# askerlee/segtran

Measured on AMD Instinct MI355X. Metric: train-step images/sec (cfg2, re-associated op order), higher is better.
Workload: dtype f32; 1 GPU; REFUGE fundus 2D, segtran eff-b4, translayers 3, layercompress 1,1,2,2, 512x512, bs 6/GPU; global_batch=6, per_gpu_batch=6, parallelism=dp1, step=fwd+BCE/Dice+bwd+allreduce+clip+BertAdam, op_order=re-associated, ranks=1

## Files before the change

include/segx.h:

```cpp
#ifndef SEGX_H
#define SEGX_H
#include <stdint.h>
#ifdef __cplusplus
extern "C" {
#endif

int segx_version(void);
int segx_last_error(char* buf, int buflen);

enum { SEGX_EPI_NONE = 0, SEGX_EPI_GELU = 1 ,
       SEGX_EPI_SWISH = 2  };
enum { SEGX_BIAS_NONE = 0, SEGX_BIAS_N = 1 , SEGX_BIAS_M = 2  };
enum { SEGX_ENGINE_F32 = 0, SEGX_ENGINE_BF16X6 = 1 };
enum { SEGX_ENGINE_SEL_DEFAULT = 0, SEGX_ENGINE_SEL_F32 = 1, SEGX_ENGINE_SEL_BF16X6 = 2 };
enum { SEGX_TILE_AUTO = 0, SEGX_TILE_128x128 = 1, SEGX_TILE_64x64 = 2, SEGX_TILE_128x32 = 3, SEGX_TILE_32x128 = 4, SEGX_TILE_64x128 = 5,
       SEGX_TILE_256x128 = 6, SEGX_TILE_WS128x128 = 7, SEGX_TILE_WS128x256 = 8, SEGX_TILE_WS64x256 = 9,
       SEGX_TILE_WS96x256 = 10, SEGX_TILE_WS256x96 = 11,
       SEGX_TILE_SKINNY_NT = 12   };
typedef struct {
    int32_t M, N, K, nb0, nb1;
    int64_t a_b0, a_b1, a_m, a_k;
    int64_t b_b0, b_b1, b_n, b_k;
    int64_t c_b0, c_b1, c_m;
    float alpha;
    int32_t epilogue, bias_mode;
    int64_t bias_b1;
    const float* bias;
    float* aux;
    float* gmax;
    float dropout_p;
    uint64_t seed, offset;
    int32_t splitk;
    float* workspace;
    int32_t tile;
    int64_t bias_b0;
    int32_t batch_reduce;
    int32_t engine;
    const void* b_planes;
    int64_t bp_b0, bp_b1;
    const float* resid;
} segx_gemm_desc;
int segx_gemm_f32(const float* A, const float* B, float* C, const segx_gemm_desc* d, void* stream);
int segx_gemm_plan(const float* A, const float* B, const segx_gemm_desc* d, int* tile, int* splitk);
int segx_gemm_plan_model(const float* A, const float* B, const segx_gemm_desc* d, int* tile, int* splitk);
int segx_gemm_route(const float* A, const float* B, const segx_gemm_desc* d, int32_t* out);
int64_t segx_x6_presplit_elems(int rows, int K, int nb0, int nb1);
int segx_x6_presplit(const float* W, int rows, int K, int64_t s_row, int64_t s_k, int nb0, int nb1, int64_t s_b0, int64_t s_b1, void* planes, void* stream);


int segx_softmax_fwd(const float* S, float* P, float* Pdrop, int64_t rows, int L, float clip, const float* gmax,
                     float p, uint64_t seed, uint64_t offset, void* stream);
// ... 229 lines not shown
```

segtran_amd/csrc/common.h:

```cpp
#pragma once
#include <hip/hip_runtime.h>
#include <stdint.h>
#include <stdio.h>
#include <stdarg.h>
#include <string.h>
#include <math.h>
#include <atomic>
#include "../../include/segx.h"

typedef float f32x16 __attribute__((ext_vector_type(16)));
typedef float f32x4 __attribute__((ext_vector_type(4)));

namespace segx {

inline char* err_buf() { static thread_local char buf[512] = {0}; return buf; }
inline int fail(int code, const char* fmt, ...) {
    va_list ap; va_start(ap, fmt); vsnprintf(err_buf(), 512, fmt, ap); va_end(ap); return code;
}
inline int check_launch(const char* what) {
    hipError_t e = hipGetLastError();
    if (e != hipSuccess) return fail((int)e, "%s: %s", what, hipGetErrorString(e));
    return 0;
}
#ifndef SEGX_MIN_WAVES_PER_SIMD
// ... 175 lines not shown
    s = odd2 ? v[0] : v[2]; r = SEGX_QUAD_XOR(s, 2); v[0] = odd2 ? r : v[0]; v[2] = odd2 ? v[2] : r;
    s = odd2 ? v[1] : v[3]; r = SEGX_QUAD_XOR(s, 2); v[1] = odd2 ? r : v[1]; v[3] = odd2 ? v[3] : r;
}
__device__ __forceinline__ float dropout_scale(uint64_t seed, uint64_t offset, uint64_t idx, float p, float inv_keep) {
    const u32x4 r = philox4(seed, (offset + idx) >> 2);
    const unsigned sel = (unsigned)((offset + idx) & 3);
    const unsigned u = sel == 0 ? r.x : sel == 1 ? r.y : sel == 2 ? r.z : r.w;
    return keep_of(u, p, inv_keep);
}

__device__ __forceinline__ float swish_fwd(float x) { return x * (1.0f / (1.0f + __expf(-x))); }
__device__ __forceinline__ float gelu_erf(float x) { return 0.5f * x * (1.0f + erff(x * 0.70710678118654752440f)); }
__device__ __forceinline__ float gelu_erf_grad(float x) {
    const float cdf = 0.5f * (1.0f + erff(x * 0.70710678118654752440f));
    const float pdf = 0.39894228040143267794f * __expf(-0.5f * x * x);
    return cdf + x * pdf;
}

#define SEGX_KNOB_TABLE(X)                                                                                                                                        \
    X(1, interp_variant, 0, 0, 2)                                                                  \
    X(2, conv_small_policy, 0, 0, 1)                          \
    X(3, bn_path, 0, 0, 2)                            \
    X(4, engine, SEGX_ENGINE_F32, SEGX_ENGINE_F32, SEGX_ENGINE_BF16X6)                                                                   \
    X(6, x6_variant, 0, 0, 7)                                      \
    X(7, conv_x6_wgrad_all, 0, 0, 2)                  \
    X(8, dw_strip_outputs, 8192, 256, 2147483647)                                                         \
    X(9, ws_grid, 256, 8, 4096)                                                                         \
    X(12, team_spin, (int)TEAM_SPIN_LIMIT, 32, 1 << 24)                                                     \
    X(13, team_drop, 0, 0, 4096)                      \
    X(14, pool_slab, 0, 0, 2)                         \
    X(15, pool_dslide, 1, 0, 1)                       \
    X(16, conv_halo, 1, 0, 1)                         \
    X(17, conv_halo_min_tiles, 256, 1, 1 << 24)         \
    X(18, skinny_nt, 1, 0, 1)                         \
    X(19, tile_walk, 1, 0, 1)                         \
    X(20, x6_terms, 6, 3, 6)
struct Knobs {
#define SEGX_KNOB_FIELD(id, field, def, lo, hi) std::atomic<int> field{def};
    SEGX_KNOB_TABLE(SEGX_KNOB_FIELD)
#undef SEGX_KNOB_FIELD
    std::atomic<int> x6_launches{0};
    std::atomic<int> x3_launches{0};
};
inline Knobs& knobs() { static Knobs k; return k; }
inline int kget(const std::atomic<int>& a) { return a.load(std::memory_order_relaxed); }

inline const uint64_t*& rng_base() { static const uint64_t* p = nullptr; return p; }

inline int ceil_div(int64_t a, int64_t b) { return (int)((a + b - 1) / b); }
__device__ __forceinline__ unsigned xcd_block(unsigned b, unsigned n) {
    const unsigned q = n >> 3, r = n & 7, xcd = b & 7, idx = b >> 3;
    return (xcd < r ? xcd * (q + 1) : r * (q + 1) + (xcd - r) * q) + idx;
}
__host__ __device__ inline int64_t i64min(int64_t a, int64_t b) { return a < b ? a : b; }
__host__ __device__ inline int64_t i64max(int64_t a, int64_t b) { return a > b ? a : b; }

struct FastDiv { unsigned d, magic; };
__host__ __device__ inline FastDiv make_fastdiv(int d) { FastDiv f; f.d = (unsigned)d; f.magic = d <= 1 ? 0u : (unsigned)(((1ull << 32) + d - 1) / d); return f; }
__device__ __forceinline__ int fdiv(int n, const FastDiv& f) {
    if (f.d <= 1) return n;
    const unsigned q = __umulhi((unsigned)n, f.magic);
    return (int)(q - (q * f.d > (unsigned)n ? 1u : 0u));
}


}
```

segtran_amd/csrc/gemm.hip:

```cpp
#include "gemm_x6ws.h"
#include "gemm_skinny.h"
#include "gemm_tuned.h"

namespace segx {

template <class Cfg, bool AKC, bool BKC, bool VEC, int EPI>
__global__ __launch_bounds__(256, 2) void gemm_f32_kernel(GemmArgs g) {
    __shared__ __attribute__((aligned(16))) TileLdsT<Cfg> lds;
    const TileCoord t = tile_coord<Cfg>(g);
    const DenseLoader<AKC, VEC, Cfg::BM> la{g.A + t.z0 * g.a_b0 + t.z1 * g.a_b1, g.a_m, g.a_k, t.m0, g.M};
    const DenseLoader<BKC, VEC, Cfg::BN> lb{g.B + t.z0 * g.b_b0 + t.z1 * g.b_b1, g.b_n, g.b_k, t.n0, g.N};
    f32x16 acc[Cfg::MI][Cfg::NJ];
    gemm_mainloop<Cfg>(acc, la, lb, t.kbeg, t.kend, lds);
    gemm_epilogue<EPI, Cfg>(acc, g, t);
}

template <class Cfg, bool AKC, bool BKC, int EPI, int WPE, int VAR = 0, int TERMS = 6>
__global__ __launch_bounds__(256) SEGX_MIN_WAVES_PER_SIMD(WPE) void gemm_x6_kernel(GemmArgs g) {
    __shared__ __attribute__((aligned(16))) unsigned char lds[X6Lds<Cfg, TERMS>::BYTES];
    const TileCoord t = tile_coord<Cfg>(g);
    const DenseLoader6<AKC, Cfg::BM> la{g.A + t.z0 * g.a_b0 + t.z1 * g.a_b1, g.a_m, g.a_k, t.m0, g.M};
    const DenseLoader6<BKC, Cfg::BN> lb{g.B + t.z0 * g.b_b0 + t.z1 * g.b_b1, g.b_n, g.b_k, t.n0, g.N};
    f32x16 acc[Cfg::MI][Cfg::NJ];
    gemm_mainloop_x6<Cfg, DenseLoader6<AKC, Cfg::BM>, DenseLoader6<BKC, Cfg::BN>, VAR, TERMS>(acc, la, lb, t.kbeg, t.kend, lds);
    gemm_epilogue<EPI, Cfg>(acc, g, t);
}

template <class Cfg, bool AKC, bool BKC, int EPI, int WPE, int TERMS = 6>
__global__ __launch_bounds__(256) SEGX_MIN_WAVES_PER_SIMD(WPE) void gemm_x6_lean_kernel(GemmArgs g) {
    __shared__ __attribute__((aligned(16))) unsigned char lds[X6Lds<Cfg, TERMS>::BYTES];
    const TileCoord t = tile_coord<Cfg>(g);
    WsDense6<AKC, Cfg::BM> la; WsDense6<BKC, Cfg::BN> lb;
    la.begin(g.A + t.z0 * g.a_b0 + t.z1 * g.a_b1, g.a_m, g.a_k, t.m0, g.M, threadIdx.x);
    lb.begin(g.B + t.z0 * g.b_b0 + t.z1 * g.b_b1, g.b_n, g.b_k, t.n0, g.N, threadIdx.x);
// ... 87 lines not shown
        double t;
        const int sk = price(TileInfo{w6.id, w6.bm, w6.bn, w6.wg_per_cu, w6.ktile_us * fws, w6.fixed_us}, M, N, K, nbatch, may_split, splitk_fixed, kget(knobs().ws_grid), &t);
        if (t < best_t * 0.97) { best_t = t; *tile = w6.id; *splitk = sk; }
    }
}
static bool gemm_lean_ok(const segx_gemm_desc* d) {
    const bool akc = (d->a_k == 1), bkc = (d->b_k == 1);
    const int64_t a_span = akc ? (int64_t)d->M * d->a_m : (int64_t)d->K * d->a_k, b_span = bkc ? (int64_t)d->N * d->b_n : (int64_t)d->K * d->b_k;
    return d->K % BKT == 0 && a_span < (1LL << 29) && b_span < (1LL << 29);
}
static bool gemm_ws_ok(const segx_gemm_desc* d) { return !d->resid && gemm_lean_ok(d); }
static void plan(int M, int N, int K, int nbatch, bool vec, bool may_split, int splitk_fixed, int* tile, int* splitk, bool skinny_ok = true) {
    const TileInfo* cand[3]; int nc = 0;
    if (!vec) cand[nc++] = &kTiles[0];
    else if (skinny_ok && N <= 48 && M > N) cand[nc++] = &tile_info(SEGX_TILE_128x32);
    else if (skinny_ok && M <= 48) cand[nc++] = &tile_info(SEGX_TILE_32x128);
    else { cand[nc++] = &kTiles[0]; cand[nc++] = &kTiles[1]; cand[nc++] = &kTiles[2]; }
    double best_t = -1.0;
    for (int i = 0; i < nc; ++i) {
        double t;
        const int sk = price(*cand[i], M, N, K, nbatch, may_split, splitk_fixed, 0, &t);
        if (best_t < 0.0 || t < best_t * 0.97) { best_t = t; *tile = cand[i]->id; *splitk = sk; }
    }
}
static bool gemm_vec_ok(const float* A, const float* B, const segx_gemm_desc* d) {
    const bool akc = (d->a_k == 1), bkc = (d->b_k == 1);
    const bool vecA = aligned16(A) && (d->a_b0 % 4 == 0) && (d->a_b1 % 4 == 0) && ((akc ? d->a_m : d->a_k) % 4 == 0) &&
                      ((akc ? d->K : d->M) % 4 == 0);
    const bool vecB = aligned16(B) && (d->b_b0 % 4 == 0) && (d->b_b1 % 4 == 0) && ((bkc ? d->b_n : d->b_k) % 4 == 0) &&
                      ((bkc ? d->K : d->N) % 4 == 0);
    return vecA && vecB;
}
static int skinny_nt_splitk(const float* A, const float* B, const segx_gemm_desc* d) {
    if (!kget(knobs().skinny_nt) || !d->batch_reduce || d->epilogue != SEGX_EPI_NONE || d->gmax || d->resid || d->a_k != 1 || d->b_k != 1) return 0;
    if (!gemm_vec_ok(A, B, d)) return 0;
    const int nbatch = d->nb0 * d->nb1;
    const int sk = (int)i64max(1, (int64_t)kget(knobs().ws_grid) * skinny_nt_wgs_per_cu(d->M, d->N) / nbatch);
    if (!skinny_nt_shape_ok(d->M, d->N, d->K, nbatch, sk * nbatch)) return 0;
    if ((int64_t)d->M * d->a_m >= (1LL << 31) || (int64_t)d->N * d->b_n >= (1LL << 31)) return 0;
    return sk;
}

static int gemm_plan_impl(const float* A, const float* B, const segx_gemm_desc* d, int* tile, int* splitk, bool use_table) {
    SEGX_REQUIRE(A && B && d && tile && splitk && d->M > 0 && d->N > 0 && d->K > 0 && d->nb0 > 0 && d->nb1 > 0, "segx_gemm_plan: bad args");
    const bool plain = d->epilogue == SEGX_EPI_NONE, swish = d->epilogue == SEGX_EPI_SWISH;
    int t = SEGX_TILE_128x128, sk = 1;
    const bool vec = gemm_vec_ok(A, B, d);
    if (const int ssk = skinny_nt_splitk(A, B, d)) { *tile = SEGX_TILE_SKINNY_NT; *splitk = ssk; return 0; }
    if (use_table && plain && !d->gmax && x6_eligible(call_engine(d), d->M, d->N, vec)) {
        const int nbt = d->nb0 * d->nb1; const bool akc_ = d->a_k == 1, bkc_ = d->b_k == 1;
        for (const TunedGemm& e : kTunedGemm)
            if (e.M == d->M && e.N == d->N && e.K == d->K && e.nb == nbt && (e.akc != 0) == akc_ && (e.bkc != 0) == bkc_) {
                if (e.tile >= SEGX_TILE_256x128 && !gemm_ws_ok(d)) break;
                *tile = e.tile; *splitk = e.splitk;
                return 0;
            }
    }
    if (x6_eligible(call_engine(d), d->M, d->N, vec) && (plain || d->a_k == 1))
        plan6(d->M, d->N, d->K, d->nb0 * d->nb1, !plain && !swish, plain && !d->gmax, 0, gemm_ws_ok(d) && !swish, (d->a_k != 1) + (d->b_k != 1), &t, &sk);
    else plan(d->M, d->N, d->K, d->nb0 * d->nb1, vec && (plain || swish), plain && !d->gmax, 0, &t, &sk, !swish);
    *tile = t; *splitk = sk;
    return 0;
}

enum GemmFamily {
    GEMM_F32,
    GEMM_X6,
    GEMM_X6_LEAN,
    GEMM_WS,
    GEMM_WS_PRE,
    GEMM_SKINNY
};
struct GemmRoute {
    int family;
    int tile;
    bool akc, bkc;
    bool vec;
    int epi;
    int sched;
    int splitk;
    int ws_grid;
    bool walk;
    int terms;
};
static bool ws_tile_id(int tile) { return tile >= SEGX_TILE_256x128 && tile <= SEGX_TILE_WS256x96; }
static bool x3_built(const GemmRoute& r) {
    if (r.sched != 0) return false;
    const bool plain = r.epi == SEGX_EPI_NONE, conv = r.akc && !r.bkc;
    switch (r.family) {
        case GEMM_WS: return plain && r.akc && (r.tile != SEGX_TILE_WS64x256 || !r.bkc);
        case GEMM_X6: return conv && r.epi != SEGX_EPI_GELU;
        case GEMM_X6_LEAN:
            if (!plain) return r.akc;
            return conv || (r.bkc && (r.tile != SEGX_TILE_64x128 || !r.akc));
        default: return false;
    }
}

static int gemm_route(const float* A, const float* B, const segx_gemm_desc* d, GemmRoute* out) {
    GemmRoute r;
    r.akc = d->a_k == 1; r.bkc = d->b_k == 1; r.vec = gemm_vec_ok(A, B, d);
    r.epi = d->epilogue; r.sched = 0; r.splitk = d->splitk > 1 ? d->splitk : 1;
    r.ws_grid = kget(knobs().ws_grid); r.walk = kget(knobs().tile_walk) != 0; r.terms = 0;
    const int want_terms = kget(knobs().x6_terms);
    const int nbatch = d->nb0 * d->nb1;
    const bool gelu = d->epilogue == SEGX_EPI_GELU, swish = d->epilogue == SEGX_EPI_SWISH, ws_forced = ws_tile_id(d->tile);
    const int engine = call_engine(d);
    SEGX_REQUIRE(!ws_forced || engine == SEGX_ENGINE_BF16X6, "segx_gemm_f32: tile %d exists on the bf16x6 engine only", d->tile);
    int tile = d->tile;
    if (tile == SEGX_TILE_SKINNY_NT) {
        const int ssk = skinny_nt_splitk(A, B, d);
        if (ssk > 0 && r.splitk <= ssk) { r.family = GEMM_SKINNY; r.tile = tile; *out = r; return 0; }
        tile = SEGX_TILE_AUTO;
    }
    const bool ws_ok = gemm_ws_ok(d);
    const bool x6 = x6_eligible(engine, d->M, d->N, r.vec) && (!gelu || r.akc) &&
                    (tile == SEGX_TILE_AUTO || tile == SEGX_TILE_128x128 || tile == SEGX_TILE_64x128 || tile == SEGX_TILE_64x64 || ws_forced);
    if (tile == SEGX_TILE_AUTO) {
        int sk_unused = 1;
        if (x6) plan6(d->M, d->N, d->K, nbatch, gelu, false, r.splitk, ws_ok && !swish, (!r.akc) + (!r.bkc), &tile, &sk_unused);
        else plan(d->M, d->N, d->K, nbatch, r.vec && !gelu, false, r.splitk, &tile, &sk_unused, !swish);
    }
    if (swish && tile != SEGX_TILE_64x128 && tile != SEGX_TILE_64x64) tile = SEGX_TILE_128x128;
    if (ws_forced && !ws_ok) tile = SEGX_TILE_128x128;
    if ((tile == SEGX_TILE_WS96x256 && (!r.akc || gelu)) || (tile == SEGX_TILE_WS256x96 && (!r.bkc || gelu))) tile = SEGX_TILE_128x128;
    if (gelu && (tile == SEGX_TILE_WS128x256 || tile == SEGX_TILE_WS64x256)) tile = SEGX_TILE_128x128;
    const bool ws = x6 && ws_ok && ws_tile_id(tile);
    if (!r.vec || (gelu && !ws) || (ws_forced && !x6)) tile = SEGX_TILE_128x128;
    r.tile = tile;
    if (!x6) {
        SEGX_REQUIRE(!gelu || r.akc, "segx_gemm_f32: the GELU epilogue is built for a k-contiguous A operand (nn.Linear, attention fusion)");
        r.family = GEMM_F32;
    } else if (ws) {
        const int v = kget(knobs().x6_variant);
        r.sched = v == 1 ? 1 : 0;
#ifdef SEGX_BENCH
        if (v >= 2 && v <= 5 && !gelu && r.akc && r.bkc) r.sched = v;
#endif
        const bool pre = d->b_planes && !gelu && (tile == SEGX_TILE_256x128 || tile == SEGX_TILE_WS128x256);
        r.family = pre ? GEMM_WS_PRE : GEMM_WS;
        if (pre) r.sched = 0;
    } else {
        const int v = kget(knobs().x6_variant);
        if (v > 0 && !gelu && r.akc && r.bkc && tile == SEGX_TILE_128x128) {
            r.family = GEMM_X6; r.sched = v;
// ... 151 lines not shown
        case GEMM_WS: return ws_kernel(r);
        case GEMM_WS_PRE: return r.tile == SEGX_TILE_256x128 ? ws_pre_tile<Cfg256x128>(r) : ws_pre_tile<Cfg128x256>(r);
        default: return f32_kernel(r);
    }
}
static void set_tiles(GemmArgs& g, const GemmLaunch& k, const GemmRoute& r) {
    g.tiles_m = ceil_div(g.M, k.bm); g.tiles_n = ceil_div(g.N, k.bn); g.mfast = r.walk ? tile_walk(g.M, g.N, g.K, g.tiles_m) : 0;
}
static int persistent_grid(const GemmArgs& g, const GemmRoute& r, int* grid) {
    const int64_t items = (int64_t)g.tiles_m * g.tiles_n * g.nbatch * g.splitk;
    SEGX_REQUIRE(items < 2147483647LL - 512, "segx_gemm_f32: too many tiles");
    *grid = (int)i64min(r.ws_grid, (items + 7) / 8 * 8);
    return 0;
}
static void slab_reduce(const segx_gemm_desc* d, float* C, const float* bias, int nslabs, bool skinny, hipStream_t stream) {
    const int64_t total = (int64_t)d->M * d->N;
    const float* ws = static_cast<const float*>(d->workspace);
    if (total * 16 <= 512 * 1024 && nslabs >= 16)
        hipLaunchKernelGGL((slab_sum_parts_kernel<16>), dim3((unsigned)((total + 15) / 16)), dim3(256), 0, stream, ws, C, bias, d->M, d->N, nslabs, total, d->c_m, d->alpha, d->bias_mode);
    else if (skinny || (total * 4 <= 1024 * 1024 && nslabs >= 4))
        hipLaunchKernelGGL((slab_sum_parts_kernel<4>), dim3((unsigned)((total + 63) / 64)), dim3(256), 0, stream, ws, C, bias, d->M, d->N, nslabs, total, d->c_m, d->alpha, d->bias_mode);
    else
        SEGX_SPLITK_REDUCE((unsigned)i64min(2048, (total + 255) / 256), stream, ws, C, bias, d->M, d->N, 1, nslabs, total, (int64_t)0, (int64_t)0, d->c_m, d->alpha,
                           d->bias_mode, (int64_t)0, (int64_t)0, total, (const float*)nullptr);
}
}

extern "C" int segx_gemm_plan(const float* A, const float* B, const segx_gemm_desc* d, int* tile, int* splitk) { return segx::gemm_plan_impl(A, B, d, tile, splitk, true); }
extern "C" int segx_gemm_plan_model(const float* A, const float* B, const segx_gemm_desc* d, int* tile, int* splitk) { return segx::gemm_plan_impl(A, B, d, tile, splitk, false); }

extern "C" int segx_gemm_route(const float* A, const float* B, const segx_gemm_desc* d, int32_t* out) {
    using namespace segx;
    SEGX_REQUIRE(A && B && d && out && d->M > 0 && d->N > 0 && d->K > 0 && d->nb0 > 0 && d->nb1 > 0, "segx_gemm_route: bad args");
    SEGX_REQUIRE(d->tile >= SEGX_TILE_AUTO && d->tile <= SEGX_TILE_SKINNY_NT && d->engine >= SEGX_ENGINE_SEL_DEFAULT && d->engine <= SEGX_ENGINE_SEL_BF16X6,
                 "segx_gemm_route: bad tile %d or engine selector %d", d->tile, d->engine);
    GemmRoute r;
    const int rc = gemm_route(A, B, d, &r);
    if (rc) return rc;
    out[0] = r.family; out[1] = r.tile; out[2] = r.terms; out[3] = r.splitk;
    return 0;
}

extern "C" int segx_gemm_f32(const float* A, const float* B, float* C, const segx_gemm_desc* d, void* stream_) {
    using namespace segx;
    hipStream_t stream = (hipStream_t)stream_;
    SEGX_REQUIRE(A && B && C && d, "segx_gemm_f32: null pointer");
    SEGX_REQUIRE(d->M > 0 && d->N > 0 && d->K > 0 && d->nb0 > 0 && d->nb1 > 0, "segx_gemm_f32: bad sizes M=%d N=%d K=%d nb=%dx%d",
                 d->M, d->N, d->K, d->nb0, d->nb1);
    SEGX_REQUIRE(d->a_m == 1 || d->a_k == 1, "segx_gemm_f32: A needs a unit stride (a_m=%lld a_k=%lld)", (long long)d->a_m, (long long)d->a_k);
    SEGX_REQUIRE(d->b_n == 1 || d->b_k == 1, "segx_gemm_f32: B needs a unit stride (b_n=%lld b_k=%lld)", (long long)d->b_n, (long long)d->b_k);
    SEGX_REQUIRE(d->epilogue == SEGX_EPI_NONE || d->epilogue == SEGX_EPI_GELU || d->epilogue == SEGX_EPI_SWISH, "segx_gemm_f32: bad epilogue %d", d->epilogue);
    SEGX_REQUIRE(d->epilogue != SEGX_EPI_SWISH || (d->a_k == 1 && d->b_n == 1 && d->b_k != 1 && !d->resid && !d->gmax && d->dropout_p == 0.f),
                 "segx_gemm_f32: the swish epilogue is built for a pointwise convolution's forward (A k-contiguous, B row-contiguous; no resid, gmax or dropout)");
    SEGX_REQUIRE(d->epilogue != SEGX_EPI_GELU || d->aux, "segx_gemm_f32: GELU epilogue needs aux");
    SEGX_REQUIRE(d->bias_mode == SEGX_BIAS_NONE || d->bias, "segx_gemm_f32: bias_mode set but bias null");
    SEGX_REQUIRE(d->dropout_p >= 0.f && d->dropout_p < 1.f, "segx_gemm_f32: dropout_p out of range");
    const int splitk = d->splitk > 1 ? d->splitk : 1;
    SEGX_REQUIRE(splitk == 1 || (d->workspace && d->epilogue == SEGX_EPI_NONE && !d->gmax), "segx_gemm_f32: split-K needs workspace and a plain epilogue");
    const bool breduce = d->batch_reduce != 0;
    SEGX_REQUIRE(!breduce || (d->workspace && d->epilogue == SEGX_EPI_NONE && !d->gmax), "segx_gemm_f32: batch_reduce needs workspace and a plain epilogue");
    SEGX_REQUIRE(!d->resid || (d->epilogue == SEGX_EPI_NONE && !breduce && !d->gmax), "segx_gemm_f32: resid needs a plain epilogue (no GELU, no batch_reduce, no gmax)");
    SEGX_REQUIRE(d->tile >= SEGX_TILE_AUTO && d->tile <= SEGX_TILE_SKINNY_NT, "segx_gemm_f32: bad tile %d", d->tile);
    SEGX_REQUIRE(d->engine >= SEGX_ENGINE_SEL_DEFAULT && d->engine <= SEGX_ENGINE_SEL_BF16X6, "segx_gemm_f32: bad engine selector %d", d->engine);
    GemmRoute r;
    int rc = gemm_route(A, B, d, &r);
    if (rc) return rc;

    const int nbatch = d->nb0 * d->nb1;
    const float* bias = d->bias_mode ? d->bias : nullptr;
    if (r.family == GEMM_SKINNY) {
        const int nslabs = splitk * nbatch;
        rc = launch_skinny_nt(A, B, static_cast<float*>(d->workspace), d->M, d->N, d->K, d->nb0, d->nb1, d->a_b0, d->a_b1, d->a_m, d->b_b0, d->b_b1, d->b_n, nslabs, stream);
        if (rc) return rc;
        slab_reduce(d, C, bias, nslabs, true, stream);
        return check_launch("segx_gemm_f32/skinny_nt_reduce");
    }
    GemmArgs g;
    g.A = A; g.B = B; g.C = C; g.bias = bias; g.aux = d->epilogue == SEGX_EPI_GELU ? d->aux : nullptr;
    g.gmax = d->gmax;
    g.M = d->M; g.N = d->N; g.K = d->K; g.nb1 = d->nb1; g.nbatch = nbatch;
    g.a_b0 = d->a_b0; g.a_b1 = d->a_b1; g.a_m = d->a_m; g.a_k = d->a_k;
    g.b_b0 = d->b_b0; g.b_b1 = d->b_b1; g.b_n = d->b_n; g.b_k = d->b_k;
    g.c_b0 = d->c_b0; g.c_b1 = d->c_b1; g.c_m = d->c_m; g.bias_b1 = d->bias_b1; g.bias_b0 = d->bias_b0;
    g.alpha = d->alpha; g.epilogue = d->epilogue; g.bias_mode = d->bias_mode;
    g.vecA = r.vec; g.vecB = r.vec;
    g.dropout_p = d->dropout_p; g.seed = d->seed; g.offset = d->offset; g.rbase = rng_base();
    g.splitk = splitk;
    g.k_chunk = splitk == 1 ? d->K : ceil_div(ceil_div(d->K, splitk), BKT) * BKT;
    g.c_split = (int64_t)nbatch * d->M * d->N;
    g.slab = breduce ? 1 : 0;
    g.Bp = nullptr; g.bp_plane = g.bp_b0 = g.bp_b1 = 0;
    if (r.family == GEMM_WS_PRE) { g.Bp = static_cast<const unsigned short*>(d->b_planes); g.bp_plane = (int64_t)d->N * d->K; g.bp_b0 = d->bp_b0; g.bp_b1 = d->bp_b1; }
    g.resid = d->resid;
    if (splitk > 1 || breduce) g.C = d->workspace;

    if (r.family != GEMM_F32) knobs().x6_launches.fetch_add(1, std::memory_order_relaxed);
    if (r.terms == 3) knobs().x3_launches.fetch_add(1, std::memory_order_relaxed);
    const GemmLaunch k = route_kernel(r);
    set_tiles(g, k, r);
    if (r.family == GEMM_WS || r.family == GEMM_WS_PRE) {
        int grid;
        rc = persistent_grid(g, r, &grid);
        if (rc) return rc;
        hipLaunchKernelGGL(k.fn, dim3(grid), dim3(512), 0, stream, g);
    } else
        hipLaunchKernelGGL(k.fn, dim3(g.tiles_m * g.tiles_n, nbatch, splitk), dim3(256), 0, stream, g);
    rc = check_launch("segx_gemm_f32");
    if (rc) return rc;
    if (breduce) {
// ... 30 lines not shown
```

segtran_amd/segx.py:

```python
import contextlib
import ctypes
import enum
import os
import torch

_HERE = os.path.dirname(os.path.abspath(__file__))
LIB_PATH = os.path.join(_HERE, 'lib', 'libsegx.so')

c_f = ctypes.c_float
c_i = ctypes.c_int32
c_l = ctypes.c_int64
c_u = ctypes.c_uint64
c_p = ctypes.c_void_p


class GemmDesc(ctypes.Structure):
    _fields_ = [('M', c_i), ('N', c_i), ('K', c_i), ('nb0', c_i), ('nb1', c_i),
                ('a_b0', c_l), ('a_b1', c_l), ('a_m', c_l), ('a_k', c_l),
                ('b_b0', c_l), ('b_b1', c_l), ('b_n', c_l), ('b_k', c_l),
                ('c_b0', c_l), ('c_b1', c_l), ('c_m', c_l),
                ('alpha', c_f), ('epilogue', c_i), ('bias_mode', c_i), ('bias_b1', c_l),
                ('bias', c_p), ('aux', c_p), ('gmax', c_p),
                ('dropout_p', c_f), ('seed', c_u), ('offset', c_u),
                ('splitk', c_i), ('workspace', c_p), ('tile', c_i), ('bias_b0', c_l), ('batch_reduce', c_i), ('engine', c_i),
                ('b_planes', c_p), ('bp_b0', c_l), ('bp_b1', c_l), ('resid', c_p)]


EPI_NONE, EPI_GELU, EPI_SWISH = 0, 1, 2
(TILE_AUTO, TILE_128x128, TILE_64x64, TILE_128x32, TILE_32x128, TILE_64x128, TILE_256x128, TILE_WS128x128, TILE_WS128x256, TILE_WS64x256,
 TILE_WS96x256, TILE_WS256x96, TILE_SKINNY_NT) = range(13)
BIAS_NONE, BIAS_N, BIAS_M = 0, 1, 2


class Knob(enum.IntEnum):
    INTERP_VARIANT = 1
    CONV_SMALL_POLICY = 2
    BN_PATH = 3
    ENGINE = 4
    X6_LAUNCHES = 5
    X6_VARIANT = 6
    CONV_X6_WGRAD_ALL = 7
    DW_STRIP_OUTPUTS = 8
    WS_GRID = 9
    TEAM_SPIN = 12
    TEAM_DROP = 13
    POOL_SLAB = 14
    POOL_DSLIDE = 15
    CONV_HALO = 16
    CONV_HALO_MIN_TILES = 17
    SKINNY_NT = 18
    TILE_WALK = 19


Knob.X6_TERMS = 20


def knob_id(name):
    v = getattr(Knob, name.upper(), None)
    if not isinstance(v, int) or name.upper().startswith('_'):
        raise KeyError(name)
    return v


# ... 105 lines not shown
        d = GemmDesc()
        d.resid = _ptr(resid)
        d.M, d.N, d.K, d.nb0, d.nb1 = M, N, K, nb[0], nb[1]
        d.a_b0, d.a_b1, d.a_m, d.a_k = a_strides
        d.b_b0, d.b_b1, d.b_n, d.b_k = b_strides
        d.c_b0, d.c_b1, d.c_m = c_strides
        d.alpha, d.epilogue, d.bias_mode, d.bias_b1, d.bias_b0 = alpha, epilogue, bias_mode, bias_b1, bias_b0
        d.bias, d.aux, d.gmax = _ptr(bias), _ptr(aux), _ptr(gmax)
        d.dropout_p, d.seed, d.offset = dropout_p, seed, offset
        if b_planes is not None:
            self._chk_t(b_planes[0])
            d.b_planes, d.bp_b0, d.bp_b1 = _ptr(b_planes[0]), b_planes[1], b_planes[2]
        d.engine = 0 if engine is None else 1 + self.ENGINES[engine]
        d.batch_reduce = 1 if batch_reduce else 0
        if splitk == 0:
            t, sk = c_i(0), c_i(0)
            self.check(self.c.segx_gemm_plan(_ptr(A), _ptr(B), ctypes.byref(d), ctypes.byref(t), ctypes.byref(sk)), 'segx_gemm_plan')
            tile, splitk = t.value, sk.value
            workspace = torch.empty(splitk * nb[0] * nb[1] * M * N, dtype=torch.float32, device=C.device) if (splitk > 1 or batch_reduce) else None
        d.splitk, d.workspace = splitk, _ptr(workspace)
        d.tile = self.force_tile if self.force_tile is not None else tile
        if self.gemm_prof is not None and C.is_cuda:
            e0, e1 = torch.cuda.Event(enable_timing=True), torch.cuda.Event(enable_timing=True)
            self.x6_launches()
            e0.record()
            rc = self.c.segx_gemm_f32(_ptr(A), _ptr(B), _ptr(C), ctypes.byref(d), self.stream(C))
            e1.record()
            self.gemm_prof.append((e0, e1, 2.0 * M * N * K * nb[0] * nb[1], (M, N, K, nb[0] * nb[1], a_strides[3] == 1, b_strides[3] == 1, splitk, d.tile),
                                   self.x6_launches() > 0))
        else:
            rc = self.c.segx_gemm_f32(_ptr(A), _ptr(B), _ptr(C), ctypes.byref(d), self.stream(C))
        self.check(rc, 'segx_gemm_f32')

    ROUTE_FAMILIES = ('f32', 'x6', 'x6_lean', 'ws', 'ws_pre', 'skinny')

    def gemm_route(self, A, B, M, N, K, a_strides, b_strides, nb=(1, 1), epilogue=EPI_NONE, splitk=1, tile=TILE_AUTO, engine=None):
        self._chk_t(A, B)
        d = GemmDesc()
        d.M, d.N, d.K, d.nb0, d.nb1 = M, N, K, nb[0], nb[1]
        d.a_b0, d.a_b1, d.a_m, d.a_k = a_strides
        d.b_b0, d.b_b1, d.b_n, d.b_k = b_strides
        d.epilogue, d.splitk, d.tile = epilogue, splitk, tile
        d.engine = 0 if engine is None else 1 + self.ENGINES[engine]
        out = (c_i * 4)()
        self.check(self.c.segx_gemm_route(_ptr(A), _ptr(B), ctypes.byref(d), out), 'segx_gemm_route')
        return self.ROUTE_FAMILIES[out[0]], out[1], out[2], out[3]

    def x6_presplit(self, W, rows, K, s_row, s_k, nb=(1, 1), s_b=(0, 0)):
        e0, e1 = (nb[0] if s_b[0] else 1), (nb[1] if s_b[1] else 1)
        planes = torch.empty(self.c.segx_x6_presplit_elems(rows, K, e0, e1), dtype=torch.int16, device=W.device)
        self._chk_t(W)
        self.check(self.c.segx_x6_presplit(_ptr(W), rows, K, s_row, s_k, e0, e1, s_b[0], s_b[1], _ptr(planes), self.stream(W)), 'segx_x6_presplit')
        per = 3 * rows * K
        return planes, (e1 * per if s_b[0] else 0), (per if s_b[1] else 0)

    def _call(self, name, ref, *args):
        conv = []
        dev = None
        hip = not self.emulated
        for a in args:
            if isinstance(a, torch.Tensor):
                if hip and not a.is_cuda:
                    raise RuntimeError('libsegx (HIP) called with a CPU tensor')
                if dev is None:
                    dev = a.device
                elif a.device != dev:
                    raise AssertionError('tensors on different devices')
# ... 494 lines not shown
```

Before: 94.68 images/s.

## Add streaming GEMM kernel for small-M/small-K shapes with N-contiguous B

Adds a streaming GEMM path for shapes with a small M or K and a long N dimension. The whole A operand stays resident in LDS while waves stream 32-column strips of B through a register prefetch ring and issue fp32 MFMA. The planner selects it automatically when the shape is eligible, enabled by a new bit in the skinny_nt knob (default now 7). The goal is to avoid the padding and low occupancy of the generic 128x128 tiles on these skinny convolution and linear shapes. The risk is that the cost heuristic or grid sizing is wrong for some shapes.

```diff
diff --git a/include/segx.h b/include/segx.h
--- a/include/segx.h
+++ b/include/segx.h
@@ -16,7 +16,8 @@
 enum { SEGX_TILE_AUTO = 0, SEGX_TILE_128x128 = 1, SEGX_TILE_64x64 = 2, SEGX_TILE_128x32 = 3, SEGX_TILE_32x128 = 4, SEGX_TILE_64x128 = 5,
        SEGX_TILE_256x128 = 6, SEGX_TILE_WS128x128 = 7, SEGX_TILE_WS128x256 = 8, SEGX_TILE_WS64x256 = 9,
        SEGX_TILE_WS96x256 = 10, SEGX_TILE_WS256x96 = 11,
-       SEGX_TILE_SKINNY_NT = 12   };
+       SEGX_TILE_SKINNY_NT = 12  ,
+       SEGX_TILE_STREAM = 13      };
 typedef struct {
     int32_t M, N, K, nb0, nb1;
     int64_t a_b0, a_b1, a_m, a_k;
diff --git a/segtran_amd/csrc/common.h b/segtran_amd/csrc/common.h
--- a/segtran_amd/csrc/common.h
+++ b/segtran_amd/csrc/common.h
@@ -231,7 +231,7 @@
     X(15, pool_dslide, 1, 0, 1)                       \
     X(16, conv_halo, 1, 0, 1)                         \
     X(17, conv_halo_min_tiles, 256, 1, 1 << 24)         \
-    X(18, skinny_nt, 1, 0, 1)                         \
+    X(18, skinny_nt, 7, 0, 7)                         \
     X(19, tile_walk, 1, 0, 1)                         \
     X(20, x6_terms, 6, 3, 6)
 struct Knobs {
diff --git a/segtran_amd/csrc/gemm.hip b/segtran_amd/csrc/gemm.hip
--- a/segtran_amd/csrc/gemm.hip
+++ b/segtran_amd/csrc/gemm.hip
@@ -1,5 +1,6 @@
 #include "gemm_x6ws.h"
 #include "gemm_skinny.h"
+#include "gemm_stream.h"
 #include "gemm_tuned.h"
 
 namespace segx {
@@ -153,7 +154,7 @@
     return vecA && vecB;
 }
 static int skinny_nt_splitk(const float* A, const float* B, const segx_gemm_desc* d) {
-    if (!kget(knobs().skinny_nt) || !d->batch_reduce || d->epilogue != SEGX_EPI_NONE || d->gmax || d->resid || d->a_k != 1 || d->b_k != 1) return 0;
+    if (!(kget(knobs().skinny_nt) & 1) || !d->batch_reduce || d->epilogue != SEGX_EPI_NONE || d->gmax || d->resid || d->a_k != 1 || d->b_k != 1) return 0;
     if (!gemm_vec_ok(A, B, d)) return 0;
     const int nbatch = d->nb0 * d->nb1;
     const int sk = (int)i64max(1, (int64_t)kget(knobs().ws_grid) * skinny_nt_wgs_per_cu(d->M, d->N) / nbatch);
@@ -161,6 +162,13 @@
     if ((int64_t)d->M * d->a_m >= (1LL << 31) || (int64_t)d->N * d->b_n >= (1LL << 31)) return 0;
     return sk;
 }
+static bool stream_ok(const float* A, const segx_gemm_desc* d) {
+    if (!(kget(knobs().skinny_nt) & 2) || d->batch_reduce || d->epilogue != SEGX_EPI_NONE || d->gmax || d->resid || d->b_n != 1) return false;
+    if (d->bias_mode != SEGX_BIAS_NONE && d->bias_mode != SEGX_BIAS_M) return false;
+    if (!stream_shape_ok(d->M, d->N, d->K, d->nb0 * d->nb1)) return false;
+    if (d->a_k == 1 && !(aligned16(A) && d->a_b0 % 4 == 0 && d->a_b1 % 4 == 0 && d->a_m % 4 == 0)) return false;
+    return (int64_t)d->K * d->b_k + d->N < (1LL << 30) && d->b_k >= 0 && 4 * d->c_m + d->N < (1LL << 30) && d->c_m >= 0;
+}
 
 static int gemm_plan_impl(const float* A, const float* B, const segx_gemm_desc* d, int* tile, int* splitk, bool use_table) {
     SEGX_REQUIRE(A && B && d && tile && splitk && d->M > 0 && d->N > 0 && d->K > 0 && d->nb0 > 0 && d->nb1 > 0, "segx_gemm_plan: bad args");
@@ -168,6 +176,7 @@
     int t = SEGX_TILE_128x128, sk = 1;
     const bool vec = gemm_vec_ok(A, B, d);
     if (const int ssk = skinny_nt_splitk(A, B, d)) { *tile = SEGX_TILE_SKINNY_NT; *splitk = ssk; return 0; }
+    if (stream_shape_pays(d->M, d->K) && stream_ok(A, d)) { *tile = SEGX_TILE_STREAM; *splitk = 1; return 0; }
     if (use_table && plain && !d->gmax && x6_eligible(call_engine(d), d->M, d->N, vec)) {
         const int nbt = d->nb0 * d->nb1; const bool akc_ = d->a_k == 1, bkc_ = d->b_k == 1;
         for (const TunedGemm& e : kTunedGemm)
@@ -190,7 +199,8 @@
     GEMM_X6_LEAN,
     GEMM_WS,
     GEMM_WS_PRE,
-    GEMM_SKINNY
+    GEMM_SKINNY,
+    GEMM_STREAM
 };
 struct GemmRoute {
     int family;
@@ -232,6 +242,10 @@
     if (tile == SEGX_TILE_SKINNY_NT) {
         const int ssk = skinny_nt_splitk(A, B, d);
         if (ssk > 0 && r.splitk <= ssk) { r.family = GEMM_SKINNY; r.tile = tile; *out = r; return 0; }
+        tile = SEGX_TILE_AUTO;
+    }
+    if (tile == SEGX_TILE_STREAM) {
+        if (r.splitk == 1 && stream_ok(A, d)) { r.family = GEMM_STREAM; r.tile = tile; r.splitk = 1; *out = r; return 0; }
         tile = SEGX_TILE_AUTO;
     }
     const bool ws_ok = gemm_ws_ok(d);
@@ -449,7 +463,7 @@
 extern "C" int segx_gemm_route(const float* A, const float* B, const segx_gemm_desc* d, int32_t* out) {
     using namespace segx;
     SEGX_REQUIRE(A && B && d && out && d->M > 0 && d->N > 0 && d->K > 0 && d->nb0 > 0 && d->nb1 > 0, "segx_gemm_route: bad args");
-    SEGX_REQUIRE(d->tile >= SEGX_TILE_AUTO && d->tile <= SEGX_TILE_SKINNY_NT && d->engine >= SEGX_ENGINE_SEL_DEFAULT && d->engine <= SEGX_ENGINE_SEL_BF16X6,
+    SEGX_REQUIRE(d->tile >= SEGX_TILE_AUTO && d->tile <= SEGX_TILE_STREAM && d->engine >= SEGX_ENGINE_SEL_DEFAULT && d->engine <= SEGX_ENGINE_SEL_BF16X6,
                  "segx_gemm_route: bad tile %d or engine selector %d", d->tile, d->engine);
     GemmRoute r;
     const int rc = gemm_route(A, B, d, &r);
@@ -477,7 +491,7 @@
     const bool breduce = d->batch_reduce != 0;
     SEGX_REQUIRE(!breduce || (d->workspace && d->epilogue == SEGX_EPI_NONE && !d->gmax), "segx_gemm_f32: batch_reduce needs workspace and a plain epilogue");
     SEGX_REQUIRE(!d->resid || (d->epilogue == SEGX_EPI_NONE && !breduce && !d->gmax), "segx_gemm_f32: resid needs a plain epilogue (no GELU, no batch_reduce, no gmax)");
-    SEGX_REQUIRE(d->tile >= SEGX_TILE_AUTO && d->tile <= SEGX_TILE_SKINNY_NT, "segx_gemm_f32: bad tile %d", d->tile);
+    SEGX_REQUIRE(d->tile >= SEGX_TILE_AUTO && d->tile <= SEGX_TILE_STREAM, "segx_gemm_f32: bad tile %d", d->tile);
     SEGX_REQUIRE(d->engine >= SEGX_ENGINE_SEL_DEFAULT && d->engine <= SEGX_ENGINE_SEL_BF16X6, "segx_gemm_f32: bad engine selector %d", d->engine);
     GemmRoute r;
     int rc = gemm_route(A, B, d, &r);
@@ -492,6 +506,9 @@
         slab_reduce(d, C, bias, nslabs, true, stream);
         return check_launch("segx_gemm_f32/skinny_nt_reduce");
     }
+    if (r.family == GEMM_STREAM)
+        return launch_stream(A, B, C, bias, d->M, d->N, d->K, d->nb0, d->nb1, d->a_b0, d->a_b1, d->a_m, d->a_k, d->b_b0, d->b_b1, d->b_k, d->c_b0, d->c_b1, d->c_m,
+                             d->bias_b0, d->bias_b1, d->alpha, stream_grid(d->M, d->N, d->K, nbatch, r.ws_grid), stream);
     GemmArgs g;
     g.A = A; g.B = B; g.C = C; g.bias = bias; g.aux = d->epilogue == SEGX_EPI_GELU ? d->aux : nullptr;
     g.gmax = d->gmax;
diff --git a/segtran_amd/csrc/gemm_stream.h b/segtran_amd/csrc/gemm_stream.h
--- /dev/null
+++ b/segtran_amd/csrc/gemm_stream.h
@@ -0,0 +1,11 @@
+#pragma once
+#include <cstdint>
+#include <hip/hip_runtime.h>
+namespace segx {
+bool stream_shape_ok(int M, int64_t N, int K, int nbatch);
+bool stream_shape_pays(int M, int K);
+int stream_grid(int M, int64_t N, int K, int nbatch, int ws_grid);
+int launch_stream(const float* A, const float* B, float* C, const float* bias, int M, int64_t N, int K, int nb0, int nb1, int64_t a_b0, int64_t a_b1, int64_t a_m,
+                  int64_t a_k, int64_t b_b0, int64_t b_b1, int64_t b_k, int64_t c_b0, int64_t c_b1, int64_t c_m, int64_t bias_b0, int64_t bias_b1, float alpha, int grid,
+                  hipStream_t stream);
+}
diff --git a/segtran_amd/csrc/gemm_stream.hip b/segtran_amd/csrc/gemm_stream.hip
--- /dev/null
+++ b/segtran_amd/csrc/gemm_stream.hip
@@ -0,0 +1,229 @@
+#include "common.h"
+#include "gemm_stream.h"
+
+namespace segx {
+
+constexpr int ST_T = 256, ST_W = ST_T / 64;
+constexpr int ST_RING = 4;
+
+struct StreamArgs {
+    const float* A; const float* B; float* C; const float* bias;
+    int M, K, nb1;
+    int upm, spm, total;
+    int per_sample;
+    int64_t a_b0, a_b1, a_m, a_k, b_b0, b_b1, b_k, c_b0, c_b1, c_m, bias_b0, bias_b1;
+    float alpha;
+};
+
+__device__ __forceinline__ void stream_fill_a(float* lds, const float* __restrict__ Az, const StreamArgs& g, int mrows, int kcn) {
+    const int slots = kcn * mrows * 2;
+    for (int s = threadIdx.x; s < slots; s += ST_T) {
+        const int h = s & 1, cm = s >> 1, c = cm / mrows, m = cm - c * mrows, k = 8 * c + 4 * h;
+        f32x4 v = f32x4{0.f, 0.f, 0.f, 0.f};
+        if (m < g.M) {
+            if (g.a_k == 1) v = *reinterpret_cast<const f32x4*>(Az + (int64_t)m * g.a_m + k);
+            else {
+                const float* p = Az + (int64_t)k * g.a_k + m;
+                v = f32x4{p[0], p[g.a_k], p[2 * g.a_k], p[3 * g.a_k]};
+            }
+        }
+        reinterpret_cast<f32x4*>(lds)[s] = v;
+    }
+}
+
+struct StreamUnit { int z0, z1, u; bool ok; };
+__device__ __forceinline__ StreamUnit stream_unit(const StreamArgs& g, int s, int w) {
+    StreamUnit t;
+    const int z = s / g.spm, u = (s - z * g.spm) * ST_W + w;
+    t.z0 = z / g.nb1; t.z1 = z - t.z0 * g.nb1;
+    t.ok = u < g.upm; t.u = t.ok ? u : g.upm - 1;
+    return t;
+}
+
+template <bool WHOLE, bool BIAS>
+__device__ __forceinline__ void stream_store_rows(const f32x16& acc, const StreamArgs& g, float* Cu, unsigned lc, const float* __restrict__ bias, int row0, int h) {
+#pragma clang fp contract(off)
+    float bv[16];
+#pragma unroll
+    for (int q = 0; q < 16; ++q) {
+        const int row = row0 + 8 * (q >> 2) + (q & 3) + 4 * h;
+        bv[q] = BIAS ? bias[WHOLE || row < g.M ? row : g.M - 1] : 0.f;
+    }
+    const int64_t step1 = g.c_m, step5 = 5 * g.c_m;
+#pragma unroll
+    for (int q = 0; q < 16; ++q) {
+        const int row = row0 + 8 * (q >> 2) + (q & 3) + 4 * h;
+        float v = acc[q] * g.alpha;
+        if (BIAS) v = v + bv[q];
+        if (WHOLE || row < g.M) ws_store<float>(ws_uniform_base_w(Cu), lc, v);
+        Cu += (q & 3) == 3 ? step5 : step1;
+    }
+}
+__device__ __forceinline__ void stream_store(const f32x16& acc, const StreamArgs& g, float* Cu, unsigned lc, const float* __restrict__ bias, int row0, int h) {
+    const bool whole = row0 + 32 <= g.M;
+    if (bias) { if (whole) stream_store_rows<true, true>(acc, g, Cu, lc, bias, row0, h); else stream_store_rows<false, true>(acc, g, Cu, lc, bias, row0, h); }
+    else { if (whole) stream_store_rows<true, false>(acc, g, Cu, lc, bias, row0, h); else stream_store_rows<false, false>(acc, g, Cu, lc, bias, row0, h); }
+}
+
+template <int FORM, int P, int LDSF>
+__global__ __launch_bounds__(ST_T) SEGX_MIN_WAVES_PER_SIMD(4) void gemm_stream_kernel(StreamArgs g) {
+    __shared__ __attribute__((aligned(16))) float lds[LDSF];
+    const int tid = threadIdx.x, lane = tid & 63, w = SEGX_WAVE_UNIFORM(tid >> 6), r = lane & 31, h = lane >> 5;
+    const int s0 = (int)((int64_t)g.total * blockIdx.x / gridDim.x), s1 = (int)((int64_t)g.total * (blockIdx.x + 1) / gridDim.x);
+    if (s0 >= s1) return;
+    const int mb = (g.M + 31) >> 5, mrows = mb * 32, kcn = g.K >> 3;
+    const int64_t bk = g.b_k, bk5 = 5 * g.b_k;
+    const unsigned lb = (unsigned)(4 * h * (int)g.b_k + r) * 4u, lc = (unsigned)(4 * h * (int)g.c_m + r) * 4u;
+    const f32x4* la = reinterpret_cast<const f32x4*>(lds) + r * 2 + h;
+    int zcur = -1;
+    auto member = [&](const StreamUnit& t) {
+        const int z = t.z0 * g.nb1 + t.z1;
+        if (z == zcur || (zcur >= 0 && !g.per_sample)) return;
+        if (zcur >= 0) __syncthreads();
+        stream_fill_a(lds, g.A + t.z0 * g.a_b0 + t.z1 * g.a_b1, g, mrows, kcn);
+        __syncthreads();
+        zcur = z;
+    };
+    auto b_of = [&](const StreamUnit& t) { return g.B + t.z0 * g.b_b0 + t.z1 * g.b_b1 + t.u * 32; };
+    auto c_of = [&](const StreamUnit& t) { return g.C + t.z0 * g.c_b0 + t.z1 * g.c_b1 + t.u * 32; };
+    auto bias_of = [&](const StreamUnit& t) { return g.bias ? g.bias + t.z0 * g.bias_b0 + t.z1 * g.bias_b1 : nullptr; };
+
+    if constexpr (FORM == 0) {
+        float nxt[P * 4];
+        auto issue = [&](int s) {
+            const float* pb = b_of(stream_unit(g, s, w));
+#pragma unroll
+            for (int j = 0; j < P * 4; ++j) {
+                nxt[j] = ws_load<float>(ws_uniform_base(pb), lb);
+                pb += (j & 3) == 3 ? bk5 : bk;
+            }
+        };
+        issue(s0);
+        for (int s = s0; s < s1; ++s) {
+            const StreamUnit t = stream_unit(g, s, w);
+            member(t);
+            float cur[P * 4];
+#pragma unroll
+            for (int j = 0; j < P * 4; ++j) { cur[j] = nxt[j]; SEGX_PIN(cur[j]); }
+            issue(s + 1 < s1 ? s + 1 : s);
+            float* Cn = c_of(t);
+            const float* __restrict__ bias = bias_of(t);
+            for (int i = 0; i < mb; ++i) {
+                f32x16 acc;
+#pragma unroll
+                for (int q = 0; q < 16; ++q) acc[q] = 0.f;
+#pragma unroll
+                for (int c = 0; c < P; ++c) {
+                    const f32x4 a = la[(c * mrows + 32 * i) * 2];
+#pragma unroll
+                    for (int e = 0; e < 4; ++e) acc = __builtin_amdgcn_mfma_f32_32x32x2f32(a[e], cur[c * 4 + e], acc, 0, 0, 0);
+                }
+                if (t.ok) stream_store(acc, g, Cn + (int64_t)(32 * i) * g.c_m, lc, bias, 32 * i, h);
+            }
+        }
+    } else {
+        float ring[ST_RING][4];
+        int ps = s0, pc = 0;
+        const float* pb = b_of(stream_unit(g, s0, w));
+        auto issue = [&](float (&slot)[4]) {
+#pragma unroll
+            for (int e = 0; e < 4; ++e) slot[e] = ws_load<float>(ws_uniform_base(pb + (8 * pc + e) * bk), lb);
+            if (pc + 1 < kcn) ++pc;
+            else if (ps + 1 < s1) { ++ps; pc = 0; pb = b_of(stream_unit(g, ps, w)); }
+        };
+#pragma unroll
+        for (int d = 0; d < ST_RING; ++d) issue(ring[d]);
+        f32x16 acc[P];
+#pragma unroll
+        for (int i = 0; i < P; ++i)
+#pragma unroll
+            for (int q = 0; q < 16; ++q) acc[i][q] = 0.f;
+        int s = s0, c = 0;
+        StreamUnit t = stream_unit(g, s0, w);
+        member(t);
+        while (s < s1) {
+#pragma unroll
+            for (int d = 0; d < ST_RING; ++d) {
+                if (s < s1) {
+                    float cur[4];
+#pragma unroll
+                    for (int e = 0; e < 4; ++e) cur[e] = ring[d][e];
+                    issue(ring[d]);
+#pragma unroll
+                    for (int i = 0; i < P; ++i) {
+                        const f32x4 a = la[(c * mrows + 32 * i) * 2];
+#pragma unroll
+                        for (int e = 0; e < 4; ++e) acc[i] = __builtin_amdgcn_mfma_f32_32x32x2f32(a[e], cur[e], acc[i], 0, 0, 0);
+                    }
+                    if (++c == kcn) {
+                        if (t.ok) {
+                            float* Cn = c_of(t);
+                            const float* __restrict__ bias = bias_of(t);
+#pragma unroll
+                            for (int i = 0; i < P; ++i) stream_store(acc[i], g, Cn + (int64_t)(32 * i) * g.c_m, lc, bias, 32 * i, h);
+                        }
+#pragma unroll
+                        for (int i = 0; i < P; ++i)
+#pragma unroll
+                            for (int q = 0; q < 16; ++q) acc[i][q] = 0.f;
+                        c = 0; ++s;
+                        if (s < s1) { t = stream_unit(g, s, w); member(t); }
+                    }
+                }
+            }
+        }
+    }
+}
+
+static int stream_form(int M, int K) {
+    if (K % 8 != 0 || M < 1) return 0;
+    if (M <= 64 && K <= 352) return 2;
+    if (K <= 64 && M <= 352) return 1;
+    return 0;
+}
+static int stream_lds_floats(int form, int M, int K) {
+    if (form == 1) return (M <= 192 ? 192 : 352) * K;
+    return (M <= 32 ? 32 : 64) * (K <= 192 ? 192 : 352);
+}
+
+bool stream_shape_ok(int M, int64_t N, int K, int nbatch) {
+    if (!stream_form(M, K) || N % 64 != 0) return false;
+    return (int64_t)nbatch * (N / 64) >= 8 && (int64_t)nbatch * ((N / 32 + ST_W - 1) / ST_W) < (1LL << 31);
+}
+
+bool stream_shape_pays(int M, int K) {
+    const int form = stream_form(M, K);
+    return form == 1 ? (M >= 96 && M <= 192) : form == 2 ? (M >= 16 && M <= 32 && K >= 96) : false;
+}
+
+int stream_grid(int M, int64_t N, int K, int nbatch, int ws_grid) {
+    const int form = stream_form(M, K);
+    const int by_regs = form == 1 ? (K <= 48 ? 4 : K <= 56 ? 3 : 2) : (M <= 32 ? 4 : 2);
+    const int per_cu = (int)i64max(1, i64min(by_regs, (160 * 1024) / (stream_lds_floats(form, M, K) * 4)));
+    return (int)i64max(1, i64min((int64_t)ws_grid * per_cu, (int64_t)nbatch * (N / 64) / 8));
+}
+
+int launch_stream(const float* A, const float* B, float* C, const float* bias, int M, int64_t N, int K, int nb0, int nb1, int64_t a_b0, int64_t a_b1, int64_t a_m,
+                  int64_t a_k, int64_t b_b0, int64_t b_b1, int64_t b_k, int64_t c_b0, int64_t c_b1, int64_t c_m, int64_t bias_b0, int64_t bias_b1, float alpha, int grid,
+                  hipStream_t stream) {
+    StreamArgs g;
+    g.A = A; g.B = B; g.C = C; g.bias = bias; g.M = M; g.K = K; g.nb1 = nb1;
+    g.upm = (int)(N / 32); g.spm = (g.upm + ST_W - 1) / ST_W; g.total = nb0 * nb1 * g.spm;
+    g.per_sample = (a_b0 != 0 || a_b1 != 0) ? 1 : 0;
+    g.a_b0 = a_b0; g.a_b1 = a_b1; g.a_m = a_m; g.a_k = a_k; g.b_b0 = b_b0; g.b_b1 = b_b1; g.b_k = b_k; g.c_b0 = c_b0; g.c_b1 = c_b1; g.c_m = c_m;
+    g.bias_b0 = bias_b0; g.bias_b1 = bias_b1; g.alpha = alpha;
+    const int form = stream_form(M, K);
+#define SEGX_STREAM(FORM_, P_, LDSF_) hipLaunchKernelGGL((gemm_stream_kernel<FORM_, P_, LDSF_>), dim3(grid), dim3(ST_T), 0, stream, g)
+#define SEGX_STREAM_WIDE(P_) case P_: if (M <= 192) SEGX_STREAM(0, P_, 192 * 8 * P_); else SEGX_STREAM(0, P_, 352 * 8 * P_); break
+    if (form == 1) switch (K / 8) { SEGX_STREAM_WIDE(1); SEGX_STREAM_WIDE(2); SEGX_STREAM_WIDE(3); SEGX_STREAM_WIDE(4); SEGX_STREAM_WIDE(5); SEGX_STREAM_WIDE(6);
+                                    SEGX_STREAM_WIDE(7); default: SEGX_STREAM_WIDE(8); }
+    else if (form == 2) {
+        if (M <= 32) { if (K <= 192) SEGX_STREAM(1, 1, 32 * 192); else SEGX_STREAM(1, 1, 32 * 352); }
+        else { if (K <= 192) SEGX_STREAM(1, 2, 64 * 192); else SEGX_STREAM(1, 2, 64 * 352); }
+    } else return fail(-1, "segx_gemm_f32/stream: M=%d K=%d is not a streaming shape", M, K);
+#undef SEGX_STREAM_WIDE
+#undef SEGX_STREAM
+    return check_launch("segx_gemm_f32/stream");
+}
+
+}
diff --git a/segtran_amd/segx.py b/segtran_amd/segx.py
--- a/segtran_amd/segx.py
+++ b/segtran_amd/segx.py
@@ -28,7 +28,7 @@
 
 EPI_NONE, EPI_GELU, EPI_SWISH = 0, 1, 2
 (TILE_AUTO, TILE_128x128, TILE_64x64, TILE_128x32, TILE_32x128, TILE_64x128, TILE_256x128, TILE_WS128x128, TILE_WS128x256, TILE_WS64x256,
- TILE_WS96x256, TILE_WS256x96, TILE_SKINNY_NT) = range(13)
+ TILE_WS96x256, TILE_WS256x96, TILE_SKINNY_NT, TILE_STREAM) = range(14)
 BIAS_NONE, BIAS_N, BIAS_M = 0, 1, 2
 
 
@@ -200,7 +200,7 @@
             rc = self.c.segx_gemm_f32(_ptr(A), _ptr(B), _ptr(C), ctypes.byref(d), self.stream(C))
         self.check(rc, 'segx_gemm_f32')
 
-    ROUTE_FAMILIES = ('f32', 'x6', 'x6_lean', 'ws', 'ws_pre', 'skinny')
+    ROUTE_FAMILIES = ('f32', 'x6', 'x6_lean', 'ws', 'ws_pre', 'skinny', 'stream')
 
     def gemm_route(self, A, B, M, N, K, a_strides, b_strides, nb=(1, 1), epilogue=EPI_NONE, splitk=1, tile=TILE_AUTO, engine=None):
         self._chk_t(A, B)
```

Result: no change. 95.08 images/s, median of 6 (+0.4%).
